# kalenforn/clip-based-cross-modal-hash

Measured on AMD Instinct MI355X. Metric: Hamming query x gallery pairs/sec (fused mAP@all pass, DCMHT COCO-shaped 64-bit), higher is better.
Workload: dtype u32; 1 GPU; configs[1] DCMHT COCO 64-bit retrieval: Q=5000 queries x R=117218 gallery items per GPU (x1 GPUs, contiguous shards), K=64 bits, C=80 classes, mAP@all; Q=5000, R_per_gpu=117218, K=64, C=80, parallelism=gallery-shard x1, query_blocks=1

## Files before the change

### clip-based-cross-modal-hash_amd/csrc/xmh_scan.hip

```cpp
#include "xmh_common.h"
#include <atomic>
#include <math.h>
#include <mutex>
#include <string.h>
#include <vector>
#include "xmh_scan_bits.h"
#include "xmh_scan_mfma.h"
#include "xmh_scan_kernels.h"

#include <stdlib.h>
#include <type_traits>

namespace {

constexpr int kSlotBudget64 = 9 * 1024;
constexpr int kSlotBudget32 = 5 * 1024;
constexpr int slots_for(int W, bool tern, int counter_bytes) {
    const int nbmax = (tern ? 64 : 32) * W + 1;
    const int budget = counter_bytes == 8 ? kSlotBudget64 : kSlotBudget32;
    const int cap = W > 8 ? 64 : 8;
    int S = 2;
    while (S < cap && nbmax * (64 / S) * counter_bytes > budget) S *= 2;
    return S;
}
// ... 62 lines not shown
WsLayout ws_layout(const xmh_scan_plan& p, size_t cache_bytes) {
    WsLayout L;
    const size_t cells = (size_t)p.nchunk * p.nbuckets * p.qpad;
    size_t o = 0;
    auto take = [&](size_t bytes) {
        const size_t at = o;
        o += (bytes + 255) & ~(size_t)255;
        return at;
    };
    L.chunk_hist = take(cells * 4);
    L.below = take(cells * 8);
    L.tot = take((size_t)p.nbuckets * p.qpad * 8);
    L.dpre = take((size_t)p.nbuckets * p.qpad * 8);
    L.cap = take((size_t)p.qpad * 4);
    L.tick = take((size_t)p.nqtile * 4);
    L.gate = take(256 + 8 * 4096);
    L.ap_part = take((size_t)p.nchunk * p.qpad * 4);
    L.pair_cache = take(cache_bytes);
    L.total = o;
    return L;
}

size_t cache_for_workspace(const xmh_scan_plan& p, int K, bool ternary, Family f, size_t ws_bytes) {
    const size_t c = pair_cache_bytes(p, K, ternary, f);
    return c && ws_bytes < ws_layout(p, c).total ? 0 : c;
}

int make_plan(int64_t Q, int64_t R, int K, int ternary, xmh_scan_plan* p, const Overrides& ov = {}) {
    if (Q <= 0 || R <= 0 || K <= 0) return xmh::fail(XMH_EINVAL, "scan plan: bad shape Q=%lld R=%lld K=%d", (long long)Q, (long long)R, K);
    if (R >= (1ll << 24) || Q >= (1ll << 24)) return xmh::fail(XMH_ENOTSUP, "scan plan: shard too large (R=%lld, Q=%lld)", (long long)R, (long long)Q);
    const int64_t nb = ternary ? 2 * (int64_t)K + 1 : (int64_t)K + 1;
    const int Wd = (K + 31) / 32;
    if (Wd > 64 || (ternary && Wd > 8))
        return xmh::fail(XMH_ENOTSUP, "scan plan: K=%d%s (at most 2048 code bits, 256 with zero planes)", K, ternary ? " ternary" : "");
    const int S64 = slots_for(instance_words(Wd), ternary != 0, 8);
    const int64_t lds_ap = nb * (64 / S64) * 8;
    if (lds_ap > 150 * 1024) return xmh::fail(XMH_ENOTSUP, "scan plan: %lld distance buckets need %lld B of LDS per wave; K=%d%s", (long long)nb, (long long)lds_ap, K, ternary ? " ternary" : "");
    const Family fam = pass1_family(K, ternary != 0, ov);
    const bool r2 = fam == Family::kR2 || fam == Family::kR2w;
    int64_t nqt = xmh::ceil_div(Q, 64);
    const int r2q = r2_geom(K).queries();
    if (r2) {
        int64_t l = r2q;
        while (l % 64) l += r2q;
        nqt = xmh::ceil_div(nqt * 64, l) * l / 64;
    }
    const int64_t wpc = 8;
    const int64_t slots = (int64_t)xmh::device_cu_count() * wpc;
    const bool cache_shape = !ternary && K > 32 && K <= 64 && cache_cap_mb() > 0;
    const int64_t rounds = nb <= 33 ? 3 : (nb <= 65 && !cache_shape ? 2 : 1);
    int64_t nchunk = rounds * slots / nqt;
    if (S64 > 8) nchunk = nchunk * 8 / S64;
    const bool mfma = fam != Family::kValu;
    if (mfma) {
        int64_t bsets = nb <= 129 ? 6 : 3;
        if (const char* e = xmh_experiment_env("XMH_BITS_SETS")) bsets = atoi(e) > 0 ? atoi(e) : bsets;
        nchunk = bsets * xmh::device_cu_count() / nqt;
        if (r2) {
            int sets = K > 32 && K <= 64 ? 1 : 2;
            if (const char* e = xmh_experiment_env("XMH_R2_SETS")) sets = atoi(e) > 0 ? atoi(e) : sets;
            nchunk = (int64_t)sets * xmh::device_cu_count() * r2_geom(K).blocks_per_cu / (nqt * 64 / r2q);
        }
    }
    if (nchunk < 1) nchunk = 1;
    if (nchunk > 8) nchunk = (nchunk + 4) / 8 * 8;
    int64_t chunk = xmh::ceil_div(R, nchunk);
    if (chunk < kMinChunk) chunk = kMinChunk;
    if (chunk > kMaxChunk) chunk = kMaxChunk;
    chunk = xmh::ceil_div(chunk, 8) * 8;
    if (mfma) {
        chunk = xmh::ceil_div(chunk, 64) * 64;
        int64_t bits_max = kBitsMaxChunk;
        if (const char* e = xmh_experiment_env("XMH_BITS_MAX_CHUNK")) bits_max = atoll(e) / 64 * 64 > 0 ? atoll(e) / 64 * 64 : bits_max;
        if (!r2 && chunk > bits_max) {
            nchunk = xmh::ceil_div(xmh::ceil_div(R, bits_max), 8) * 8;
            chunk = xmh::ceil_div(xmh::ceil_div(R, nchunk), 64) * 64;
        }
    }
    nchunk = xmh::ceil_div(R, chunk);
    p->chunk = chunk;
    p->nchunk = nchunk;
    p->nqtile = nqt;
    p->qpad = nqt * 64;
    p->nbuckets = nb;
    p->ws_bytes = ws_layout(*p, pair_cache_bytes(*p, K, ternary != 0, fam)).total;
    return XMH_OK;
}

int lane_order_ok(hipStream_t st) {
    static int cached[64];
    static bool have[64];
    static std::mutex mu;
    int dev = 0;
    if (hipGetDevice(&dev) != hipSuccess || dev < 0 || dev >= 64) return 0;
    if (getenv("XMH_SCAN_MASKED") != nullptr) return 0;
    std::lock_guard<std::mutex> lock(mu);
    if (have[dev]) return cached[dev];
    int ok = 0;
    {
        const char* fe = getenv("XMH_SCAN_PROBE_FAULT");
        const int fault = fe && atoi(fe) != 0;
        uint32_t* flag = nullptr;
        float* sink = nullptr;
        if (hipMalloc(&flag, 8) == hipSuccess && hipMalloc(&sink, 256) == hipSuccess) {
            uint32_t h[2] = {0, 1};
            int cus = xmh::device_cu_count();
            if (hipMemsetAsync(flag, 0, 8, st) == hipSuccess) {
                hipLaunchKernelGGL(k_probe_lane_order, dim3(1), dim3(64), 0, st, flag);
                hipLaunchKernelGGL(k_probe_lane_order_load, dim3((unsigned)(cus * 25)), dim3(64), 0, st, flag + 1, fault, sink);
                if (hipGetLastError() == hipSuccess && hipMemcpyAsync(h, flag, 8, hipMemcpyDeviceToHost, st) == hipSuccess && hipStreamSynchronize(st) == hipSuccess)
                    ok = h[0] == 1u && h[1] == 0u;
            }
        }
        if (flag) (void)hipFree(flag);
        if (sink) (void)hipFree(sink);
        if (!ok)
            fprintf(stderr, "xmh: the lane-order probe FAILED on device %d%s: same-address returning LDS adds are not served in lane order here; "
                            "pass 2 runs the masked kernels (about 2x slower, same results).\n", dev, fault ? " (XMH_SCAN_PROBE_FAULT set: forced)" : "");
// ... 134 lines not shown
    s.kern = Kern::kApS; s.W = tb ? 8 : W; s.LW = LW; s.tern = tern && !tb; s.masked = masked;
    s.cache = cache && !byte128 && !masked && pair_cache_shape(s.W, s.tern);
    s.stand_in = byte128 && apc;
    s.gate = size_gate | (s.stand_in ? kByWrap : 0u) | (r.rank_bits ? kByWidth : 0u);
    for (const bool p32 : {true, false}) {
        if (p32 ? r.rank_bits == 0 : apc16) continue;
        s.p32 = p32;
        s.S = s.cache ? cache_slots(s.W) : slots_for(s.W, s.tern, p32 ? 4 : 8);
        s.NW = s.S == 64 ? waves_for(s.W, s.tern) : 1;
        r.p2[r.n2++] = s;
    }
    return r;
}

int describe_launch(const Launch& l, char* out, size_t n) {
    static const char* const tf[2] = {"false", "true"};
    auto exists = [&](auto tern_c) { return dispatch_shape<decltype(tern_c)::value>(l.W, l.LW, [](auto, auto) { return (int)XMH_OK; }); };
    switch (l.kern) {
    case Kern::kHistS:
    case Kern::kApS:
        if (const int rc = l.tern ? exists(std::true_type{}) : exists(std::false_type{})) return rc;
        if (l.kern == Kern::kHistS) snprintf(out, n, "k_scan_hist_s<%d, %d, %s, %d, %d, %s>", l.W, l.LW, tf[l.tern], l.S, l.NW, tf[l.cache]);
        else
            snprintf(out, n, "k_scan_ap_s<%d, %d, %s, %s, %d, %s, %s, %d, %s>", l.W, l.cache ? 1 : l.LW, tf[l.tern], tf[!l.cache], l.S, tf[l.p32], tf[l.masked],
                     l.NW, tf[l.cache]);
        break;
    case Kern::kHistR2:
    case Kern::kHistR2w:
        snprintf(out, n, "k_scan_hist_%s<%d, %d, %d, %s>", l.kern == Kern::kHistR2 ? "r2" : "r2w", l.nml, l.NW, l.S, tf[l.cache]);
        break;
    case Kern::kHistB: {
        int nsh, nqt;
        xmh::scan_hist_bits_shape(l.S, l.tern, &nsh, &nqt);
        snprintf(out, n, "k_scan_hist_b<%d, %d, %d, %d, %s, %s>", l.S, kMfmaWaves, nsh, nqt, tf[l.cache], tf[l.tern]);
        break;
    }
    case Kern::kApC: snprintf(out, n, "k_scan_ap_c<false, %d, %s>", l.eb, tf[l.half]); break;
    case Kern::kApR2: snprintf(out, n, "k_scan_ap_r2<%d, %d, %d, false>", l.nml, l.NW, l.S); break;
    }
    return XMH_OK;
}

int check_common(const char* who, const ScanCall& c, const xmh_scan_plan& p) {
    if (!c.qbits || !c.rbits || !c.qlab || !c.rlab || !c.ws) return xmh::fail(XMH_EINVAL, "%s: null pointer", who);
    if ((c.qzero == nullptr) != (c.rzero == nullptr)) return xmh::fail(XMH_EINVAL, "%s: zero masks must be given for both sides or neither", who);
    if (c.C <= 0) return xmh::fail(XMH_EINVAL, "%s: C=%d", who, c.C);
    const size_t need = ws_layout(p, 0).total;
    if (c.ws_bytes < need) return xmh::fail(XMH_EINVAL, "%s: workspace too small (%zu < %zu; %zu with the pair cache)", who, c.ws_bytes, need, (size_t)p.ws_bytes);
    return XMH_OK;
}

ScanArgs make_args(const ScanCall& c, const xmh_scan_plan& p) {
    return ScanArgs{c.qbits, c.qzero, c.qlab, c.rbits, c.rzero, c.rlab, (int)c.Q, (int)c.R, c.K, (int)p.chunk, (int)p.nchunk, (int)p.nqtile, (int)p.qpad,
                    (int)p.nbuckets, nullptr};
}

MfmaArgs r2_args(const ScanCall& c, const Launch& l, const xmh_scan_plan& p, int nqt) {
    MfmaArgs a{c.qbits, (int)c.Q, (int)c.R, c.K, l.W, (int)p.chunk, (int)p.nchunk, nqt, (int)p.nbuckets, (int)p.qpad};
    a.rbits = c.rbits; a.rlab = c.rlab; a.qlab = c.qlab; a.LW = l.LW;
    return a;
}

struct Geom { unsigned grid, block; size_t lds; int nqt; };
Geom launch_geom(const Launch& l, const xmh_scan_plan& p) {
    const size_t nb = (size_t)p.nbuckets;
    const bool ap = l.kern == Kern::kApS || l.kern == Kern::kApC || l.kern == Kern::kApR2;
    Geom g{0, 64u * (unsigned)l.NW, 0, 0};
    if (l.kern == Kern::kHistS || l.kern == Kern::kApS) {
        g.lds = ((nb * (64 / l.S) * (ap && !l.p32 ? 2 : 1) + 3) & ~(size_t)3) * 4 * l.NW + (ap && l.cache ? 0 : aos_ring_bytes(l.W, l.LW, l.tern));
        g.nqt = (int)p.nqtile * l.S / l.NW;
    } else if (l.kern == Kern::kApC) {
        g.lds = nb * (64 / l.S) * 8; g.nqt = (int)p.nqtile * l.S;
    } else if (l.kern == Kern::kHistB) {
        g.nqt = (int)(p.qpad / (16 * kMfmaWaves));
    } else {
        g.lds = (size_t)l.NW * l.S * nb * 16 * (ap ? 8 : 4); g.nqt = (int)(p.qpad / (l.NW * l.S * 16));
    }
    g.grid = (unsigned)(8 * g.nqt * xmh::ceil_div(p.nchunk, 8));
    return g;
}

template <typename KernT, typename... Args>
int start(const char* who, const Launch& l, const Geom& g, hipStream_t st, KernT kern, int S, int NW, bool cache, Args... args) {
    if (l.S != S || l.NW != NW || l.cache != cache)
        return xmh::fail(XMH_ENOTSUP, "%s: the route names an instance with S=%d NW=%d cache=%d, the one compiled for W=%d LW=%d has S=%d NW=%d cache=%d", who, l.S,
                         l.NW, (int)l.cache, l.W, l.LW, S, NW, (int)cache);
    if (const int rc = xmh::raise_dynamic_lds(reinterpret_cast<const void*>(kern), g.lds, who)) return rc;
    hipLaunchKernelGGL(kern, dim3(g.grid), dim3(g.block), g.lds, st, args...);
    return XMH_OK;
}

struct ScanCtx {
    const ScanCall& c;
    hipStream_t st;
    xmh_scan_plan p;
    ScanRoute r;
    WsLayout L;
    ScanArgs a;
    uint32_t kcap = 0xffffffffu;
    bool capped = false;
    template <typename T> T* at(size_t off) const { return reinterpret_cast<T*>(static_cast<char*>(c.ws) + off); }
    uint32_t* chunk_hist() const { return at<uint32_t>(L.chunk_hist); }
    const uint2* below() const { return at<uint2>(L.below); }
    uint2* tot() const { return at<uint2>(L.tot); }
    uint2* dpre() const { return at<uint2>(L.dpre); }
    uint32_t* cap_ws() const { return at<uint32_t>(L.cap); }
    float* ap_part() const { return at<float>(L.ap_part); }
    ScanArgs args(const Geom& g, bool cached) const { ScanArgs as = a; as.nqt = g.nqt; as.pair_cache = cached ? pair_cache() : nullptr; return as; }
    uint32_t* gate(int word = 0) const { return at<uint32_t>(L.gate) + word; }
    const uint32_t* gate_if(const Launch& l, unsigned g, int word) const { return (l.gate & g) ? gate(word) : nullptr; }
    uint4* pair_cache() const { return r.cache_bytes ? at<uint4>(L.pair_cache) : nullptr; }
};

int plan_call(const char* who, ScanCtx& x, const Overrides& ov) {
    if (const int rc = make_plan(x.c.Q, x.c.R, x.c.K, x.c.tern, &x.p, ov)) return rc;
    return check_common(who, x.c, x.p);
}
void route_call(ScanCtx& x, Mode mode, const Overrides& ov) {
    x.r = scan_route(x.p, x.c, mode, ov, x.st);
    x.a = make_args(x.c, x.p);
    x.L = ws_layout(x.p, x.r.cache_bytes);
}

int valu_hist(const ScanCtx& x) {
    const Launch& h = x.r.p1;
    const Geom g = launch_geom(h, x.p);
    const ScanArgs as = x.args(g, h.cache);
    auto go = [&](auto kern, int S, int NW, bool cache) {
        xmh::ProfScope prof("scan_hist", x.st);
        return start("xmh_hamming_hist", h, g, x.st, kern, S, NW, cache, as, x.chunk_hist());
    };
    auto launch = [&](auto tern_c) {
        constexpr bool T = decltype(tern_c)::value;
        return dispatch_shape<T>(h.W, h.LW, [&](auto w, auto l) {
            constexpr int WW = decltype(w)::value, LL = decltype(l)::value;
            if constexpr (kPairCacheShape<WW, T>) {
                if (h.cache) return go(k_scan_hist_s<WW, LL, T, cache_slots(WW), 1, true>, cache_slots(WW), 1, true);
            }
            constexpr int S = slots_for(WW, T, 4);
            constexpr int NW = S == 64 ? waves_for(WW, T) : 1;
            return go(k_scan_hist_s<WW, LL, T, S, NW, false>, S, NW, false);
        });
    };
    return h.tern ? launch(std::true_type{}) : launch(std::false_type{});
}

int mfma_hist(const ScanCtx& x) {
    const Launch& h = x.r.p1;
    const xmh_scan_plan& p = x.p;
    const Geom g = launch_geom(h, p);
    uint32_t* chunk_hist = x.chunk_hist();
    uint4* cache = x.pair_cache();
    if (h.kern == Kern::kHistB) {
        xmh::ScanBitsArgs a{x.c.rbits, x.c.rlab, x.c.qbits, x.c.qlab, (int)x.c.Q, (int)x.c.R, x.c.K, h.W, h.LW, (int)p.chunk, (int)p.nchunk, g.nqt,
                            (int)p.nbuckets, (int)p.qpad};
        a.rzero = x.c.rzero; a.qzero = x.c.qzero;
        return xmh::launch_scan_hist_bits(a, h.S, chunk_hist, cache, x.st);
    }
    hipLaunchKernelGGL(k_scan_touch, dim3((unsigned)(8 * kTouchPerChunk * xmh::ceil_div(p.nchunk, 8))), dim3(256), 0, x.st, x.c.rbits, x.c.rlab, x.c.R, h.W, h.LW,
                       p.chunk, (int)p.nchunk, x.at<uint32_t>(x.L.tick), (int)((x.L.gate + 256 - x.L.tick) / 4));
    XMH_LAUNCH_CHECK("xmh_hamming_hist control words");
    const MfmaArgs a = r2_args(x.c, h, p, g.nqt);
    xmh::ProfScope prof("scan_hist", x.st);
    auto go = [&](auto kern, int NW, int NQ, bool cached, auto... wrap_word) { return start("xmh_hamming_hist", h, g, x.st, kern, NQ, NW, cached, a, chunk_hist, cache, wrap_word...); };
    if (h.kern == Kern::kHistR2w) {
        uint32_t* ovf = x.gate(kGateWrapped);
        return h.nml == 1 ? (h.cache ? go(k_scan_hist_r2w<1, 4, 2, true>, 4, 2, true, ovf) : go(k_scan_hist_r2w<1, 4, 2, false>, 4, 2, false, ovf))
                          : (h.cache ? go(k_scan_hist_r2w<2, 4, 2, true>, 4, 2, true, ovf) : go(k_scan_hist_r2w<2, 4, 2, false>, 4, 2, false, ovf));
    }
    return h.nml == 1 ? (h.cache ? go(k_scan_hist_r2<1, 4, 4, true>, 4, 4, true) : go(k_scan_hist_r2<1, 4, 4, false>, 4, 4, false))
                      : (h.cache ? go(k_scan_hist_r2<2, 4, 4, true>, 4, 4, true) : go(k_scan_hist_r2<2, 4, 4, false>, 4, 4, false));
}

int hamming_hist_impl(const ScanCall& c, uint32_t* hist_all, uint32_t* hist_rel, xmh_stream_t stream, const Overrides& ov) {
    ScanCtx x{c, xmh::as_stream(stream)};
    if (const int rc = plan_call("xmh_hamming_hist", x, ov)) return rc;
    route_call(x, Mode::kUnsharded, ov);
    const xmh_scan_plan& p = x.p;
    const Kern kern = x.r.p1.kern;
    if (kern == Kern::kHistS || kern == Kern::kHistB) XMH_HIP(hipMemsetAsync(x.at<char>(x.L.tick), 0, x.L.gate + 256 - x.L.tick, x.st));
    if (const int rc = kern == Kern::kHistS ? valu_hist(x) : mfma_hist(x)) return rc;
    XMH_LAUNCH_CHECK("xmh_hamming_hist");
    hipLaunchKernelGGL(k_scan_below, dim3((unsigned)p.nqtile, (unsigned)xmh::ceil_div(p.nbuckets, 4)), dim3(256), 0, x.st, x.chunk_hist(), (int)p.qpad,
                       (int)p.nbuckets, (int)p.nchunk, kern != Kern::kHistS ? kRelHi16 : 0u, x.at<uint2>(x.L.below), x.tot(), x.at<uint32_t>(x.L.tick), (int)c.Q, x.dpre(),
                       x.cap_ws(), x.gate(), hist_all, hist_rel);
    XMH_LAUNCH_CHECK("xmh_hamming_hist below");
    return XMH_OK;
}

}

extern "C" int xmh_scan_plan_make(int64_t Q, int64_t R, int K, int ternary, xmh_scan_plan* plan_host) {
    if (!plan_host) return xmh::fail(XMH_EINVAL, "xmh_scan_plan_make: null plan");
    return make_plan(Q, R, K, ternary, plan_host);
}

extern "C" size_t xmh_scan_pair_cache_bytes(int64_t Q, int64_t R, int K, int ternary) {
    xmh_scan_plan p;
    if (make_plan(Q, R, K, ternary, &p)) return 0;
    return pair_cache_bytes(p, K, ternary != 0, pass1_family(K, ternary != 0, {}));
}

extern "C" size_t xmh_scan_pair_cache_offset(int64_t Q, int64_t R, int K, int ternary) {
    xmh_scan_plan p;
    if (make_plan(Q, R, K, ternary, &p)) return (size_t)-1;
    return ws_layout(p, 0).pair_cache;
}

extern "C" size_t xmh_scan_ws_bytes_nocache(int64_t Q, int64_t R, int K, int ternary) {
    xmh_scan_plan p;
    if (make_plan(Q, R, K, ternary, &p)) return 0;
    return ws_layout(p, 0).total;
}

extern "C" int xmh_scan_describe(int64_t Q, int64_t R, int K, int C, int ternary, char* out, size_t out_bytes) {
    if (!out || out_bytes < 64) return xmh::fail(XMH_EINVAL, "xmh_scan_describe: buffer too small");
    xmh_scan_plan p;
    if (const int rc = make_plan(Q, R, K, ternary, &p)) return rc;
    Overrides ov;
    ov.describe = true;
    const ScanCall c{nullptr, nullptr, nullptr, nullptr, nullptr, nullptr, Q, R, K, C, nullptr, (size_t)p.ws_bytes, ternary != 0};
    const ScanRoute r = scan_route(p, c, Mode::kUnsharded, ov, nullptr);
    char p1[160], p2[200] = "", one[120];
    if (const int rc = describe_launch(r.p1, p1, sizeof(p1))) return rc;
    for (const bool p32 : {true, false})
        for (int i = 0; i < r.n2; ++i) {
            if (r.p2[i].stand_in || r.p2[i].p32 != p32) continue;
            if (const int rc = describe_launch(r.p2[i], one, sizeof(one))) return rc;
            const size_t at = strlen(p2);
            snprintf(p2 + at, sizeof(p2) - at, "%s%s", at ? "|" : "", one);
        }
    if ((size_t)snprintf(out, out_bytes, "pass1=%s;pass2=%s", p1, p2) >= out_bytes) return xmh::fail(XMH_EINVAL, "xmh_scan_describe: buffer too small");
    return XMH_OK;
}

extern "C" int xmh_hamming_hist(const uint32_t* qbits, const uint32_t* qzero, const uint32_t* qlab,
                                const uint32_t* rbits, const uint32_t* rzero, const uint32_t* rlab, int64_t Q, int64_t R,
                                int K, int C, void* ws, size_t ws_bytes, uint32_t* hist_all, uint32_t* hist_rel,
                                xmh_stream_t stream) {
    XMH_RANGE("xmh_hamming_hist (pass 1)");
    const ScanCall c{qbits, qzero, qlab, rbits, rzero, rlab, Q, R, K, C, ws, ws_bytes, qzero != nullptr};
    return hamming_hist_impl(c, hist_all, hist_rel, stream, {});
}

namespace {
int ap_offsets(const ScanCtx& x, const Pass2& o) {
    const xmh_scan_plan& p = x.p;
    if (o.mode == Mode::kUnsharded) return XMH_OK;
    if (o.mode == Mode::kAllToAll)
        hipLaunchKernelGGL(k_shard_scatter_offsets, dim3((unsigned)xmh::ceil_div(p.qpad, 256), (unsigned)p.nbuckets + 1), dim3(256), 0, x.st,
                           reinterpret_cast<const uint2*>(o.hist_g), (int)p.nbuckets, (int)(p.qpad / o.world), (int)x.c.Q, (int)p.qpad, o.k, x.dpre(), x.cap_ws(),
                           o.cap, x.gate(2));
    else if (o.mode == Mode::kTotals)
        hipLaunchKernelGGL(k_shard_offsets_dpre, dim3((unsigned)p.nqtile), dim3(256), 0, x.st, reinterpret_cast<const uint2*>(o.hist_g), o.world, o.rank,
                           (int)x.c.Q, (int)p.qpad, (int)p.nbuckets, o.k, x.dpre(), x.cap_ws(), o.cap, x.gate(2));
    else
        hipLaunchKernelGGL(k_scan_dpre, dim3((unsigned)p.nqtile), dim3(256), 0, x.st, (const uint2*)x.tot(), (int)x.c.Q, (int)p.qpad, (int)p.nbuckets, o.base_all,
                           o.base_rel, o.nrel_total, o.k, x.dpre(), x.cap_ws(), o.cap, (uint32_t*)nullptr, (uint32_t*)nullptr, (uint32_t*)nullptr, x.gate(2));
    XMH_LAUNCH_CHECK(o.mode == Mode::kAllToAll ? "xmh_hamming_map_sharded_offsets scatter" : (o.mode == Mode::kTotals ? "xmh_hamming_map_sharded offsets" : "xmh_hamming_ap dpre"));
    return XMH_OK;
}

int ap_launch_c(const ScanCtx& x, const Launch& l) {
    const Geom g = launch_geom(l, x.p);
    const ScanArgs as = x.args(g, true);
    xmh::ProfScope prof("scan_ap", x.st);
    auto go = [&](auto kc, int S) {
        return start("xmh_hamming_ap", l, g, x.st, kc, S, 1, l.cache, as, x.below(), (const uint2*)x.dpre(), (const uint32_t*)x.cap_ws(), x.ap_part(),
                     x.gate_if(l, kBySize, 2), x.kcap, x.gate_if(l, kByWrap, kGateWrapped), x.gate_if(l, kByWidth, 0), l.gate & kByWidth ? x.r.rank_bits : 0);
    };
    if (l.eb == 16) return x.capped ? go(k_scan_ap_c<true, 16>, 8) : go(k_scan_ap_c<false, 16>, 8);
    if (l.half) return x.capped ? go(k_scan_ap_c<true, 8, true>, 8) : go(k_scan_ap_c<false, 8, true>, 8);
    return x.capped ? go(k_scan_ap_c<true, 8>, 4) : go(k_scan_ap_c<false, 8>, 4);
}

int ap_launch_r2(const ScanCtx& x, const Launch& l) {
    const Geom g = launch_geom(l, x.p);
    const MfmaArgs ma = r2_args(x.c, l, x.p, g.nqt);
    xmh::ProfScope prof("scan_ap", x.st);
    auto go = [&](auto kern) {
        return start("xmh_hamming_ap", l, g, x.st, kern, kAp2Groups, kAp2Waves, l.cache, ma, x.below(), (const uint2*)x.dpre(), (const uint32_t*)x.cap_ws(), x.ap_part(),
                     x.gate_if(l, kBySize, 2), x.kcap);
    };
    return l.nml == 1 ? (x.capped ? go(k_scan_ap_r2<1, kAp2Waves, kAp2Groups, true>) : go(k_scan_ap_r2<1, kAp2Waves, kAp2Groups, false>))
                      : (x.capped ? go(k_scan_ap_r2<2, kAp2Waves, kAp2Groups, true>) : go(k_scan_ap_r2<2, kAp2Waves, kAp2Groups, false>));
}

int ap_launch_s(const ScanCtx& x, const Launch& l) {
    const Geom g = launch_geom(l, x.p);
    const ScanArgs as = x.args(g, l.cache);
    auto go = [&](auto kern, int S, int NW, bool cache, const uint32_t* run_if) {
        xmh::ProfScope prof(l.p32 ? "scan_ap32" : "scan_ap", x.st);
        return start("xmh_hamming_ap", l, g, x.st, kern, S, NW, cache, as, x.below(), (const uint2*)x.dpre(), (const uint32_t*)x.cap_ws(), x.ap_part(),
                     (const uint32_t*)x.gate(), x.r.rank_bits, x.kcap, x.gate_if(l, kBySize, 2), run_if);
    };
    auto by_shape = [&](auto tern_c, auto cap_c, auto p32_c, auto masked_c) {
        constexpr bool T = decltype(tern_c)::value, CP = decltype(cap_c)::value, P32 = decltype(p32_c)::value, MK = decltype(masked_c)::value;
        return dispatch_shape<T>(l.W, l.LW, [&](auto w, auto lw) {
            constexpr int WW = decltype(w)::value, LL = decltype(lw)::value;
            if constexpr (P32 && MK) return xmh::fail(XMH_ENOTSUP, "xmh_hamming_ap: the masked fallback runs 64-bit counters only");
            else {
                if constexpr (kPairCacheShape<WW, T> && !MK) {
                    if (l.cache)
                        return go(k_scan_ap_s<WW, 1, T, CP, cache_slots(WW), P32, MK, 1, true>, cache_slots(WW), 1, true, nullptr);
                }
                (void)CP;
                constexpr int S = slots_for(WW, T, P32 ? 4 : 8);
                constexpr int NW = S == 64 ? waves_for(WW, T) : 1;
                return go(k_scan_ap_s<WW, LL, T, true, S, P32, MK, NW, false>, S, NW, false, x.gate_if(l, kByWrap, kGateWrapped));
            }
        });
    };
    using T1 = std::true_type; using T0 = std::false_type;
    auto by_mask = [&](auto t, auto c, auto w) { return l.masked ? by_shape(t, c, w, T1{}) : by_shape(t, c, w, T0{}); };
    auto by_width = [&](auto t, auto c) { return l.p32 ? by_mask(t, c, T1{}) : by_mask(t, c, T0{}); };
    auto by_cap = [&](auto t) { return x.capped ? by_width(t, T1{}) : by_width(t, T0{}); };
    return l.tern ? by_cap(T1{}) : by_cap(T0{});
}

int ap_reduce(const ScanCtx& x, const Pass2& o) {
    const int64_t Q = x.c.Q;
    const unsigned nred = (unsigned)xmh::ceil_div(Q, 64);
    if (o.map_out && nred <= 4096) {
        hipLaunchKernelGGL(k_ap_reduce_map, dim3(nred), dim3(256), 0, x.st, (const float*)x.ap_part(), (int)Q, (int)x.p.qpad, (int)x.p.nchunk,
                           (const uint32_t*)x.cap_ws(), x.kcap, o.cap, o.ap_sum, x.at<double>(x.L.gate + 256), x.gate(1), o.map_out);
        XMH_LAUNCH_CHECK("xmh_hamming_map reduce+finalize");
        return XMH_OK;
    }
    hipLaunchKernelGGL(k_ap_reduce, dim3(nred), dim3(256), 0, x.st, (const float*)x.ap_part(), (int)Q, (int)x.p.qpad, (int)x.p.nchunk, o.ap_sum,
                       o.mode != Mode::kUnsharded ? (const uint32_t*)nullptr : (const uint32_t*)x.cap_ws(), x.kcap, o.cap);
    XMH_LAUNCH_CHECK("xmh_hamming_ap reduce");
    if (o.map_out) {
        hipLaunchKernelGGL(k_map_finalize, dim3(1), dim3(256), 0, x.st, (const double*)o.ap_sum, (const int32_t*)o.cap, Q, o.map_out);
        XMH_LAUNCH_CHECK("xmh_hamming_map finalize");
    }
    return XMH_OK;
}

static std::atomic<int> g_verify{0};
constexpr int XMH_EVERIFY_CODE = -74;

int hamming_ap_impl(const ScanCall& c, const Pass2& o, xmh_stream_t stream, const Overrides& ov);
// ... 237 lines not shown
```

### clip-based-cross-modal-hash_amd/csrc/xmh_scan_mfma.h

```cpp
#pragma once
#include "xmh_common.h"
#include <type_traits>

namespace {

constexpr int kMaxChunk = 32768;
constexpr uint32_t kF23 = 0x4B000000u;
constexpr int64_t kFloatBitsMaxItems = (1ll << 23) - 3;
constexpr int kMinChunk = 256;

struct ScanArgs {
    const uint32_t* qbits;
    const uint32_t* qzero;
    const uint32_t* qlab;
    const uint32_t* rbits;
    const uint32_t* rzero;
    const uint32_t* rlab;
    int Q, R, K;
    int chunk, nchunk, nqt, qpad, nb;
    uint4* pair_cache;
};

__device__ __forceinline__ bool map_block(const ScanArgs& a, int& chunk_id, int& qtile) {
    const int b = blockIdx.x;
    const int xcd = b & 7;
    const int t = b >> 3;
    qtile = t % a.nqt;
    chunk_id = xcd + 8 * (t / a.nqt);
    return chunk_id < a.nchunk;
}

typedef int v4i __attribute__((ext_vector_type(4)));

struct MfmaArgs {
    const uint32_t* qbits;
    int Q, R, K, W;
    int chunk, nchunk, nqt, nb, qpad;
    const uint32_t* rbits = nullptr;
    const uint32_t* rlab = nullptr;
    const uint32_t* qlab = nullptr;
    int LW = 0;
};

__device__ __forceinline__ bool mfma_map_block(const MfmaArgs& a, int& chunk_id, int& qtile) {
    const int b = blockIdx.x;
    const int xcd = b & 7, t = b >> 3;
    qtile = t % a.nqt;
    chunk_id = xcd + 8 * (t / a.nqt);
    return chunk_id < a.nchunk;
}

__device__ __forceinline__ v4i label_query_f4(uint32_t w, uint32_t one) {
    v4i r;
#pragma unroll
    for (int j = 0; j < 4; ++j) r[j] = (int)(((w >> j) & 0x11111111u) * one);
    return r;
}
__device__ __forceinline__ v4i label_item_f4(uint32_t w) {
    return v4i{(int)(w & 0x11111111u), (int)(w & 0x22222222u), (int)(w & 0x44444444u), (int)((w >> 1) & 0x44444444u)};
}

template <int NML, int NW, int NQ, bool CACHE>
__device__ __forceinline__ void scan_hist_r2_body(const MfmaArgs& a, uint32_t* __restrict__ chunk_hist, uint4* __restrict__ pair_cache) {
    static_assert(NML == 1 || NML == 2, "one i8 label tile (at most 64 classes) or one FP4 label tile (65-128 classes)");
    constexpr bool F4 = NML == 2;
    constexpr int NMI = 2, NMQ = 3;
    constexpr bool REGS = true;
    extern __shared__ __attribute__((aligned(16))) uint32_t lds[];
    int chunk_id, qtile;
    if (!mfma_map_block(a, chunk_id, qtile)) return;
    const int lane = threadIdx.x & 63, wave = threadIdx.x >> 6;
    const int ql = lane & 15, slot = lane >> 4;
    const int t16 = (qtile * NW + wave) * NQ;
    const int ncell = a.nb * 16;
    uint32_t* cnt = lds + (wave * NQ) * ncell;
    for (int e = lane; e < NQ * ncell; e += 64) cnt[e] = 0u;
    v4i bq[NQ][NMQ], cq[NQ], kqv[REGS ? NQ : 1];
    bool valid[NQ];
    const int rsh = 4 * (slot & 1), rwi = slot >> 1;
#pragma unroll
    for (int h = 0; h < NQ; ++h) {
        valid[h] = (t16 + h) * 16 + ql < a.Q;
        int pcq = 0;
        {
            const int64_t q = (int64_t)(t16 + h) * 16 + ql;
            uint32_t qw = 0u;
            if (valid[h]) {
                for (int w = 0; w < a.W; ++w) pcq += __popc(a.qbits[q * a.W + w]);
                if (rwi < a.W) qw = a.qbits[q * a.W + rwi];
            }
            qw >>= rsh;
#pragma unroll
            for (int j = 0; j < 4; ++j) {
                const uint32_t t = (qw >> j) & 0x01010101u;
                const bool on = valid[h] && rwi < a.W;
                if (j & 1) {
                    bq[h][0][j] = on ? (int)(0x20202020u ^ (t * 0xc0u)) : 0;
                    bq[h][1][j] = on ? (int)(0x01010101u ^ (t * 0xfeu)) : 0;
                } else {
                    bq[h][0][j] = on ? (int)(0x40404040u ^ (t << 7)) : 0;
                    bq[h][1][j] = on ? (int)(0x02020202u ^ (t * 0xfcu)) : 0;
                }
            }
            if constexpr (F4) {
                bq[h][2] = label_query_f4(valid[h] && slot < a.LW ? a.qlab[q * a.LW + slot] : 0u, 0x2u);
            } else {
                uint32_t lw = 0u;
                if (valid[h] && rwi < a.LW) lw = a.qlab[q * a.LW + rwi];
                lw >>= rsh;
#pragma unroll
                for (int j = 0; j < 4; ++j) bq[h][2][j] = (int)((lw >> j) & 0x01010101u);
            }
            const int k2 = 2 * pcq;
            kqv[h] = v4i{k2, k2, k2, k2};
        }
        const int c0 = (int)(uint32_t)(uintptr_t)(__attribute__((address_space(3))) uint32_t*)(cnt + h * ncell) + ql * 4 + (valid[h] ? 64 * pcq : 0);
        cq[h] = v4i{c0, c0, c0, c0};
    }
    v4i lab0 = {0x10000, 0x10000, 0x10000, 0x10000};
    asm volatile("" : "+v"(lab0));
#pragma unroll
    for (int h = 0; h < NQ; ++h) asm volatile("" : "+v"(cq[h]));
#pragma unroll
// ... 206 lines not shown
        build(A[3], wcur[3]);
#ifdef XMH_ABL_NOBUILD
        }
#endif
        group(std::integral_constant<int, 0>{});
        group(std::integral_constant<int, 1>{});
        group(std::integral_constant<int, 2>{});
        group(std::integral_constant<int, 3>{});
        asm volatile(XMH_R2_TAIL ::: "memory");
        consume(cw[NQ - 1][3], A[3]);
#ifdef XMH_ABL_NOSTORE
        if (CACHE && a.Q < 0) {
#else
        if (CACHE) {
#endif
#pragma unroll
            for (int h = 0; h < NQ; ++h) {
                uint4* dst = crow[h] + (int64_t)i * 64;
                __builtin_nontemporal_store(cw[h][0], &dst->x);
                __builtin_nontemporal_store(cw[h][1], &dst->y);
                __builtin_nontemporal_store(cw[h][2], &dst->z);
                __builtin_nontemporal_store(cw[h][3], &dst->w);
            }
        }
#pragma unroll
        for (int g = 0; g < 4; ++g)
#pragma unroll
            for (int m = 0; m < NMI; ++m) wcur[g][m] = wnxt[g][m];
    }
    const int npad = nbat * 64 - (int)(hi - lo);
    asm volatile("s_waitcnt lgkmcnt(0)" ::: "memory");
    if (npad > 0 && slot == 0) {
#pragma unroll
        for (int h = 0; h < NQ; ++h) {
            if (!valid[h]) continue;
            const int64_t q = (int64_t)(t16 + h) * 16 + ql;
            int dpad = 0;
            for (int w = 0; w < a.W; ++w) dpad += __popc(a.qbits[q * a.W + w]);
            cnt[h * ncell + dpad * 16 + ql] -= (uint32_t)npad << 16;
        }
    }
#pragma unroll
    for (int h = 0; h < NQ; ++h) {
        uint32_t* __restrict__ out = chunk_hist + ((int64_t)chunk_id * a.nb) * a.qpad + (t16 + h) * 16;
        for (int e = lane; e < ncell; e += 64) out[(int64_t)(e >> 4) * a.qpad + (e & 15)] = cnt[h * ncell + e];
    }
}

constexpr int kTouchPerChunk = 8;
__global__ __launch_bounds__(256) void k_scan_touch(const uint32_t* __restrict__ rbits, const uint32_t* __restrict__ rlab, int64_t R, int W, int LW, int64_t chunk,
                                                    int nchunk, uint32_t* __restrict__ ctl, int ctl_words) {
    if (blockIdx.x == 0)
        for (int e = threadIdx.x; e < ctl_words; e += 256) ctl[e] = 0u;
    const int b = blockIdx.x;
    const int c = (b & 7) + 8 * ((b >> 3) / kTouchPerChunk), sub = (b >> 3) % kTouchPerChunk;
    if (c >= nchunk) return;
    const int64_t lo = (int64_t)c * chunk, hi = lo + chunk < R ? lo + chunk : R;
    uint32_t acc = 0u;
    auto sweep = [&](const uint32_t* base, int64_t w0, int64_t w1) {
        for (int64_t w = w0 + ((int64_t)sub * 256 + threadIdx.x) * 32; w < w1; w += (int64_t)kTouchPerChunk * 256 * 32) acc ^= base[w];
    };
    sweep(rbits, lo * W, hi * W);
    sweep(rlab, lo * LW, hi * LW);
    asm volatile("" ::"v"(acc));
}

#ifndef XMH_R2_ATTR
#define XMH_R2_ATTR
#endif
template <int NML, int NW, int NQ, bool CACHE>
__global__ __launch_bounds__(64 * NW) XMH_R2_ATTR void k_scan_hist_r2(MfmaArgs a, uint32_t* __restrict__ chunk_hist, uint4* __restrict__ pair_cache) {
    scan_hist_r2_body<NML, NW, NQ, CACHE>(a, chunk_hist, pair_cache);
}

#define XMH_W_MFMA(D, A, B, C) "v_mfma_i32_16x16x64_i8 %[" D "], %[" A "], %[" B "], %[" C "]\n\t"
#define XMH_W_MFMA_F4(D, A, B, C) "v_mfma_f32_16x16x128_f8f6f4 %[" D "], %[" A "], %[" B "], %[" C "] cbsz:4 blgp:4\n\t"
#define XMH_W_MIN(I, L) "v_min_u32 %[" I "], 0x10001, %[" L "]\n\t"
#define XMH_W_ADD(A, D) "ds_add_u32 %[" A "], %[" D "]\n\t"
#define XMH_W_FUSED_CACHE(LAB) \
    asm volatile("s_nop 3\n\t" LAB("lab", "al0", "bl0", "lab0") XMH_W_MIN("i0", "lp0") XMH_W_MIN("i1", "lp1") XMH_W_MIN("i2", "lp2")                \
                 XMH_W_MIN("i3", "lp3") XMH_W_ADD("ap0", "i0") XMH_W_MFMA("addr", "a0", "ba0", "cq") XMH_W_ADD("ap1", "i1")                         \
                 XMH_W_MFMA("addr", "a1", "ba1", "addr") XMH_W_ADD("ap2", "i2") XMH_W_MFMA("d2", "a0", "bd0", "kq") XMH_W_ADD("ap3", "i3")          \
                 XMH_W_MFMA("d2", "a1", "bd1", "d2")                                                                                                \
                 : [lab] "=&v"(lab), [addr] "=&v"(addr), [d2] "=&v"(d2), [i0] "=&v"(i0), [i1] "=&v"(i1), [i2] "=&v"(i2), [i3] "=&v"(i3)             \
                 : [a0] "v"(At[0]), [a1] "v"(At[1]), [al0] "v"(At[2]), [ba0] "v"(bA[h][0]), [ba1] "v"(bA[h][1]), [bd0] "v"(bD[h][0]),               \
                   [bd1] "v"(bD[h][1]), [bl0] "v"(bL[h]), [lab0] "v"(lab0), [cq] "v"(cq[h]), [kq] "v"(kq[h]), [lp0] "v"(lab_p[0]),                  \
                   [lp1] "v"(lab_p[1]), [lp2] "v"(lab_p[2]), [lp3] "v"(lab_p[3]), [ap0] "v"(addr_p[0]), [ap1] "v"(addr_p[1]), [ap2] "v"(addr_p[2]), \
                   [ap3] "v"(addr_p[3])                                                                                                             \
                 : "memory")
#define XMH_W_FUSED_PLAIN(LAB) \
    asm volatile("s_nop 3\n\t" LAB("lab", "al0", "bl0", "lab0") XMH_W_MIN("i0", "lp0") XMH_W_MIN("i1", "lp1") XMH_W_MIN("i2", "lp2")                 \
                 XMH_W_MIN("i3", "lp3") XMH_W_ADD("ap0", "i0") XMH_W_ADD("ap1", "i1") XMH_W_MFMA("addr", "a0", "ba0", "cq") XMH_W_ADD("ap2", "i2")   \
                 XMH_W_ADD("ap3", "i3") XMH_W_MFMA("addr", "a1", "ba1", "addr")                                                                      \
                 : [lab] "=&v"(lab), [addr] "=&v"(addr), [i0] "=&v"(i0), [i1] "=&v"(i1), [i2] "=&v"(i2), [i3] "=&v"(i3)                              \
                 : [a0] "v"(At[0]), [a1] "v"(At[1]), [al0] "v"(At[2]), [ba0] "v"(bA[h][0]), [ba1] "v"(bA[h][1]), [bl0] "v"(bL[h]), [lab0] "v"(lab0), \
                   [cq] "v"(cq[h]), [lp0] "v"(lab_p[0]), [lp1] "v"(lab_p[1]), [lp2] "v"(lab_p[2]), [lp3] "v"(lab_p[3]), [ap0] "v"(addr_p[0]),        \
                   [ap1] "v"(addr_p[1]), [ap2] "v"(addr_p[2]), [ap3] "v"(addr_p[3])                                                                  \
                 : "memory")
template <int NML, int NW, int NQ, bool CACHE>
__global__ __launch_bounds__(64 * NW) void k_scan_hist_r2w(MfmaArgs a, uint32_t* __restrict__ chunk_hist, uint4* __restrict__ pair_cache,
                                                           uint32_t* __restrict__ ovf) {
    static_assert(NML == 1 || NML == 2, "one i8 label tile (at most 64 classes) or one FP4 label tile (65-128 classes)");
    constexpr bool F4 = NML == 2;
    constexpr int NMC = 2, NMI = NMC + 1;
    extern __shared__ __attribute__((aligned(16))) uint32_t lds[];
    int chunk_id, qtile;
    if (!mfma_map_block(a, chunk_id, qtile)) return;
    const int lane = threadIdx.x & 63, wave = threadIdx.x >> 6;
    const int ql = lane & 15, slot = lane >> 4;
    const int t16 = (qtile * NW + wave) * NQ;
    const int ncell = a.nb * 16;
    uint32_t* cnt = lds + (wave * NQ) * ncell;
    for (int e = lane; e < NQ * ncell; e += 64) cnt[e] = 0u;
    const int rsh = 4 * (slot & 1), rwi = slot >> 1;
    v4i bA[NQ][NMC], bD[NQ][NMC], bL[NQ], cq[NQ], kq[NQ];
    bool valid[NQ];
#pragma unroll
    for (int h = 0; h < NQ; ++h) {
        const int64_t q = (int64_t)(t16 + h) * 16 + ql;
        valid[h] = q < a.Q;
        int pcq = 0;
        if (valid[h])
            for (int w = 0; w < a.W; ++w) pcq += __popc(a.qbits[q * a.W + w]);
#pragma unroll
        for (int c = 0; c < NMC; ++c) {
            const int wi = 2 * c + rwi;
            const bool on = valid[h] && wi < a.W;
            const uint32_t qw = (on ? a.qbits[q * a.W + wi] : 0u) >> rsh;
#pragma unroll
            for (int j = 0; j < 4; ++j) {
                const uint32_t t = (qw >> j) & 0x01010101u;
                if (j & 1) {
                    bA[h][c][j] = on ? (int)(0x20202020u ^ (t * 0xc0u)) : 0;
                    bD[h][c][j] = on ? (int)(0x01010101u ^ (t * 0xfeu)) : 0;
                } else {
                    bA[h][c][j] = on ? (int)(0x40404040u ^ (t << 7)) : 0;
                    bD[h][c][j] = on ? (int)(0x02020202u ^ (t * 0xfcu)) : 0;
                }
            }
        }
        if constexpr (F4) {
            bL[h] = label_query_f4(valid[h] && slot < a.LW ? a.qlab[q * a.LW + slot] : 0u, 0x2u);
        } else {
            uint32_t lw = 0u;
            if (valid[h] && rwi < a.LW) lw = a.qlab[q * a.LW + rwi];
            lw >>= rsh;
#pragma unroll
            for (int j = 0; j < 4; ++j) bL[h][j] = (int)((lw >> j) & 0x01010101u);
        }
        const int c0 = (int)(uint32_t)(uintptr_t)(__attribute__((address_space(3))) uint32_t*)(cnt + h * ncell) + ql * 4 + (valid[h] ? 64 * pcq : 0);
        const int k2 = valid[h] ? 2 * pcq : 0;
        cq[h] = v4i{c0, c0, c0, c0};
        kq[h] = v4i{k2, k2, k2, k2};
    }
    v4i lab0 = {0x10000, 0x10000, 0x10000, 0x10000};
    asm volatile("" : "+v"(lab0));
#pragma unroll
    for (int h = 0; h < NQ; ++h) asm volatile("" : "+v"(cq[h]), "+v"(kq[h]));
    const int64_t lo = (int64_t)chunk_id * a.chunk;
    const int64_t hi = (lo + a.chunk < a.R) ? lo + a.chunk : a.R;
// ... 395 lines not shown
            issue4(oldB, mB, r3);
            r3 = words_at(bi + 7);
            drain8(oldA, mA);
            drain0(oldB, mB);
        }
        const int rem = nfull - bi;
        if (rem >= 2) {
            issue4(oldA, mA, r0);
            issue4(oldB, mB, r1);
            drain8(oldA, mA);
            drain0(oldB, mB);
            if (rem == 3) {
                issue4(oldA, mA, r2);
                drain0(oldA, mA);
            }
        } else if (rem == 1) {
            issue4(oldA, mA, r0);
            drain0(oldA, mA);
        }
        cw = rem == 0 ? r0 : (rem == 1 ? r1 : (rem == 2 ? r2 : r3));
    }
    const int cntb = (int)(hi - lo) - nfull * 64;
    slow_batch(cw, cntb);
#pragma unroll
    for (int o = QW; o < 64; o <<= 1) acc += __shfl_xor(acc, o, 64);
    if (slot == 0) ap_part[(int64_t)chunk_id * a.qpad + q] = acc;
}

#define XMH_AP2_SETA "v113", "v115", "v117", "v119", "v[112:113]", "v[114:115]", "v[116:117]", "v[118:119]"
#define XMH_AP2_SETB "v121", "v123", "v125", "v127", "v[120:121]", "v[122:123]", "v[124:125]", "v[126:127]"
#define XMH_AP2_MFMA(D, A, B, C) "v_mfma_i32_16x16x64_i8 %[" D "], %[" A "], %[" B "], " C "\n\t"
#define XMH_AP2_MFMA_F4(D, A, B, C) "v_mfma_f32_16x16x128_f8f6f4 %[" D "], %[" A "], %[" B "], " C " cbsz:4 blgp:4\n\t"
#define XMH_AP2_MAX(H, L) "v_max_i32 " H ", -1, %[" L "]\n\t"
#define XMH_AP2_ADD(O, A, P) "ds_add_rtn_u64 %[" O "], %[" A "], " P "\n\t"
#define XMH_AP2_FUSED_(LAB, H0, H1, H2, H3, P0, P1, P2, P3)                                                                              \
    "s_nop 3\n\t" LAB("lab", "a1", "q1", "0") XMH_AP2_MAX(H0, "l0") XMH_AP2_MAX(H1, "l1") XMH_AP2_MAX(H2, "l2") XMH_AP2_MAX(H3, "l3")    \
    XMH_AP2_MFMA("addr", "a0", "q0", "%[c0]") XMH_AP2_ADD("o0", "p0", P0) XMH_AP2_ADD("o1", "p1", P1) XMH_AP2_ADD("o2", "p2", P2)       \
    XMH_AP2_ADD("o3", "p3", P3)
#define XMH_AP2_TAIL_(H0, H1, H2, H3, P0, P1, P2, P3)                                                                                     \
    XMH_AP2_MAX(H0, "l0") XMH_AP2_MAX(H1, "l1") XMH_AP2_MAX(H2, "l2") XMH_AP2_MAX(H3, "l3") XMH_AP2_ADD("o0", "p0", P0)                   \
    XMH_AP2_ADD("o1", "p1", P1) XMH_AP2_ADD("o2", "p2", P2) XMH_AP2_ADD("o3", "p3", P3)
#define XMH_AP2_FUSED(...) XMH_AP2_FUSED_(__VA_ARGS__)
#define XMH_AP2_TAIL(...) XMH_AP2_TAIL_(__VA_ARGS__)
template <int NML, int NW, int NQ, bool CAPPED>
__global__ __launch_bounds__(64 * NW) void k_scan_ap_r2(MfmaArgs a, const uint2* __restrict__ below, const uint2* __restrict__ dpre,
                                                        const uint32_t* __restrict__ cap_ws, float* __restrict__ ap_part,
                                                        const uint32_t* __restrict__ items_total, uint32_t kcap) {
    using u64 = unsigned long long;
    static_assert(NML == 1 || NML == 2, "one i8 label tile (at most 64 classes) or one FP4 label tile (65-128 classes)");
    constexpr bool F4 = NML == 2;
    constexpr int NMI = 2;
    extern __shared__ __attribute__((aligned(16))) uint32_t lds[];
    int chunk_id, qtile;
    if (!mfma_map_block(a, chunk_id, qtile)) return;
    if (items_total && (int64_t)*items_total > kFloatBitsMaxItems) return;
    const int lane = threadIdx.x & 63, wave = threadIdx.x >> 6;
    const int ql = lane & 15, slot = lane >> 4;
    const int t16 = (qtile * NW + wave) * NQ;
    const int ncell = a.nb * 16;
    u64* cnt = reinterpret_cast<u64*>(lds) + (wave * NQ) * ncell;
    auto pack = [](uint2 x, uint2 y) {
        return (u64)(kF23 + x.x + y.x + 1u) | ((u64)(kF23 + (0x7fffffu - (x.y + y.y + 1u))) << 32);
    };
#pragma unroll
    for (int h = 0; h < NQ; ++h) {
        const uint2* __restrict__ pb = below + ((int64_t)chunk_id * a.nb) * a.qpad + (t16 + h) * 16;
        const uint2* __restrict__ pd = dpre + (t16 + h) * 16;
        u64* c = cnt + h * ncell;
        auto cell = [&](int e) { return e; };
        int e = lane;
        for (; e + 3 * 64 < ncell; e += 4 * 64) {
            uint2 x[4], y[4];
#pragma unroll
            for (int j = 0; j < 4; ++j) {
                const int ee = e + j * 64;
                const int64_t at = (int64_t)(ee >> 4) * a.qpad + (ee & 15);
                x[j] = pb[at];
                y[j] = pd[at];
            }
#pragma unroll
            for (int j = 0; j < 4; ++j) c[cell(e + j * 64)] = pack(x[j], y[j]);
        }
        for (; e < ncell; e += 64) {
            const int64_t at = (int64_t)(e >> 4) * a.qpad + (e & 15);
            c[cell(e)] = pack(pb[at], pd[at]);
        }
    }
    v4i bq[NQ], bl[NQ], cq[NQ];
    float capf[NQ], acc[NQ];
    const int rsh = 4 * (slot & 1), rwi = slot >> 1;
#pragma unroll
    for (int h = 0; h < NQ; ++h) {
        const int64_t q = (int64_t)(t16 + h) * 16 + ql;
        const bool valid = q < a.Q;
        int pcq = 0;
        uint32_t qw = 0u;
        if (valid) {
            for (int w = 0; w < a.W; ++w) pcq += __popc(a.qbits[q * a.W + w]);
            if (rwi < a.W) qw = a.qbits[q * a.W + rwi];
        }
        qw >>= rsh;
        const bool on = valid && rwi < a.W;
#pragma unroll
        for (int j = 0; j < 4; ++j) {
            const uint32_t t = (qw >> j) & 0x01010101u;
            if (j & 1) bq[h][j] = on ? (int)(0x20202020u ^ (t * 0xc0u)) : 0;
            else bq[h][j] = on ? (int)(0x40404040u ^ (t << 7)) : 0;
// ... 184 lines not shown
```

Before: 1761 billion pairs/s.

## Map blocks exactly to chunks and skip all-padding query tiles in AP pass

Replaces the XCD-strided block mapping, which rounded the grid up to a multiple of 8 chunks and launched idle blocks, with a shared map that covers whole groups of 8 chunks XCD-strided and then places the remaining tail chunks linearly. The AP launches now size their grid to the query tiles that actually contain queries rather than all padded tiles, so blocks on padding do no work. An opt-in env flag also lets the R2 plan keep a non-multiple-of-8 chunk count. The tail chunks lose the XCD-aligned placement, which may hurt L2 locality for them, and the touch kernel uses a single part per tail chunk.

```diff
diff --git a/clip-based-cross-modal-hash_amd/csrc/xmh_scan.hip b/clip-based-cross-modal-hash_amd/csrc/xmh_scan.hip
--- a/clip-based-cross-modal-hash_amd/csrc/xmh_scan.hip
+++ b/clip-based-cross-modal-hash_amd/csrc/xmh_scan.hip
@@ -138,6 +138,7 @@
     int64_t nchunk = rounds * slots / nqt;
     if (S64 > 8) nchunk = nchunk * 8 / S64;
     const bool mfma = fam != Family::kValu;
+    bool fill = false;
     if (mfma) {
         int64_t bsets = nb <= 129 ? 6 : 3;
         if (const char* e = xmh_experiment_env("XMH_BITS_SETS")) bsets = atoi(e) > 0 ? atoi(e) : bsets;
@@ -146,10 +147,11 @@
             int sets = K > 32 && K <= 64 ? 1 : 2;
             if (const char* e = xmh_experiment_env("XMH_R2_SETS")) sets = atoi(e) > 0 ? atoi(e) : sets;
             nchunk = (int64_t)sets * xmh::device_cu_count() * r2_geom(K).blocks_per_cu / (nqt * 64 / r2q);
+            if (const char* e = xmh_experiment_env("XMH_R2_FILL")) fill = atoi(e) != 0 && fam == Family::kR2 && sets == 1 && cache_shape && ap_r2_mode() != 1;
         }
     }
     if (nchunk < 1) nchunk = 1;
-    if (nchunk > 8) nchunk = (nchunk + 4) / 8 * 8;
+    if (nchunk > 8 && !fill) nchunk = (nchunk + 4) / 8 * 8;
     int64_t chunk = xmh::ceil_div(R, nchunk);
     if (chunk < kMinChunk) chunk = kMinChunk;
     if (chunk > kMaxChunk) chunk = kMaxChunk;
@@ -390,7 +392,7 @@
 
 ScanArgs make_args(const ScanCall& c, const xmh_scan_plan& p) {
     return ScanArgs{c.qbits, c.qzero, c.qlab, c.rbits, c.rzero, c.rlab, (int)c.Q, (int)c.R, c.K, (int)p.chunk, (int)p.nchunk, (int)p.nqtile, (int)p.qpad,
-                    (int)p.nbuckets, nullptr};
+                    (int)p.nbuckets, nullptr, (int)p.nqtile};
 }
 
 MfmaArgs r2_args(const ScanCall& c, const Launch& l, const xmh_scan_plan& p, int nqt) {
@@ -399,8 +401,8 @@
     return a;
 }
 
-struct Geom { unsigned grid, block; size_t lds; int nqt; };
-Geom launch_geom(const Launch& l, const xmh_scan_plan& p) {
+struct Geom { unsigned grid, block; size_t lds; int nqt, nrun; };
+Geom launch_geom(const Launch& l, const xmh_scan_plan& p, int64_t Q) {
     const size_t nb = (size_t)p.nbuckets;
     const bool ap = l.kern == Kern::kApS || l.kern == Kern::kApC || l.kern == Kern::kApR2;
     Geom g{0, 64u * (unsigned)l.NW, 0, 0};
@@ -414,7 +416,12 @@
     } else {
         g.lds = (size_t)l.NW * l.S * nb * 16 * (ap ? 8 : 4); g.nqt = (int)(p.qpad / (l.NW * l.S * 16));
     }
-    g.grid = (unsigned)(8 * g.nqt * xmh::ceil_div(p.nchunk, 8));
+    g.nrun = g.nqt;
+    if (ap) {
+        static const bool all_tiles = xmh_experiment_env("XMH_AP_TILES") && atoi(xmh_experiment_env("XMH_AP_TILES")) == 0;
+        if (!all_tiles) g.nrun = (int)xmh::ceil_div(Q, p.qpad / g.nqt);
+    }
+    g.grid = xmh::scan_grid_blocks(g.nrun, (int)p.nchunk);
     return g;
 }
 
@@ -444,7 +451,7 @@
     uint2* dpre() const { return at<uint2>(L.dpre); }
     uint32_t* cap_ws() const { return at<uint32_t>(L.cap); }
     float* ap_part() const { return at<float>(L.ap_part); }
-    ScanArgs args(const Geom& g, bool cached) const { ScanArgs as = a; as.nqt = g.nqt; as.pair_cache = cached ? pair_cache() : nullptr; return as; }
+    ScanArgs args(const Geom& g, bool cached) const { ScanArgs as = a; as.nqt = g.nqt; as.nrun = g.nrun; as.pair_cache = cached ? pair_cache() : nullptr; return as; }
     uint32_t* gate(int word = 0) const { return at<uint32_t>(L.gate) + word; }
     const uint32_t* gate_if(const Launch& l, unsigned g, int word) const { return (l.gate & g) ? gate(word) : nullptr; }
     uint4* pair_cache() const { return r.cache_bytes ? at<uint4>(L.pair_cache) : nullptr; }
@@ -462,7 +469,7 @@
 
 int valu_hist(const ScanCtx& x) {
     const Launch& h = x.r.p1;
-    const Geom g = launch_geom(h, x.p);
+    const Geom g = launch_geom(h, x.p, x.c.Q);
     const ScanArgs as = x.args(g, h.cache);
     auto go = [&](auto kern, int S, int NW, bool cache) {
         xmh::ProfScope prof("scan_hist", x.st);
@@ -486,7 +493,7 @@
 int mfma_hist(const ScanCtx& x) {
     const Launch& h = x.r.p1;
     const xmh_scan_plan& p = x.p;
-    const Geom g = launch_geom(h, p);
+    const Geom g = launch_geom(h, p, x.c.Q);
     uint32_t* chunk_hist = x.chunk_hist();
     uint4* cache = x.pair_cache();
     if (h.kern == Kern::kHistB) {
@@ -495,7 +502,7 @@
         a.rzero = x.c.rzero; a.qzero = x.c.qzero;
         return xmh::launch_scan_hist_bits(a, h.S, chunk_hist, cache, x.st);
     }
-    hipLaunchKernelGGL(k_scan_touch, dim3((unsigned)(8 * kTouchPerChunk * xmh::ceil_div(p.nchunk, 8))), dim3(256), 0, x.st, x.c.rbits, x.c.rlab, x.c.R, h.W, h.LW,
+    hipLaunchKernelGGL(k_scan_touch, dim3(xmh::scan_grid_blocks(kTouchPerChunk, (int)p.nchunk)), dim3(256), 0, x.st, x.c.rbits, x.c.rlab, x.c.R, h.W, h.LW,
                        p.chunk, (int)p.nchunk, x.at<uint32_t>(x.L.tick), (int)((x.L.gate + 256 - x.L.tick) / 4));
     XMH_LAUNCH_CHECK("xmh_hamming_hist control words");
     const MfmaArgs a = r2_args(x.c, h, p, g.nqt);
@@ -600,7 +607,7 @@
 }
 
 int ap_launch_c(const ScanCtx& x, const Launch& l) {
-    const Geom g = launch_geom(l, x.p);
+    const Geom g = launch_geom(l, x.p, x.c.Q);
     const ScanArgs as = x.args(g, true);
     xmh::ProfScope prof("scan_ap", x.st);
     auto go = [&](auto kc, int S) {
@@ -613,8 +620,8 @@
 }
 
 int ap_launch_r2(const ScanCtx& x, const Launch& l) {
-    const Geom g = launch_geom(l, x.p);
-    const MfmaArgs ma = r2_args(x.c, l, x.p, g.nqt);
+    const Geom g = launch_geom(l, x.p, x.c.Q);
+    const MfmaArgs ma = r2_args(x.c, l, x.p, g.nrun);
     xmh::ProfScope prof("scan_ap", x.st);
     auto go = [&](auto kern) {
         return start("xmh_hamming_ap", l, g, x.st, kern, kAp2Groups, kAp2Waves, l.cache, ma, x.below(), (const uint2*)x.dpre(), (const uint32_t*)x.cap_ws(), x.ap_part(),
@@ -625,7 +632,7 @@
 }
 
 int ap_launch_s(const ScanCtx& x, const Launch& l) {
-    const Geom g = launch_geom(l, x.p);
+    const Geom g = launch_geom(l, x.p, x.c.Q);
     const ScanArgs as = x.args(g, l.cache);
     auto go = [&](auto kern, int S, int NW, bool cache, const uint32_t* run_if) {
         xmh::ProfScope prof(l.p32 ? "scan_ap32" : "scan_ap", x.st);
diff --git a/clip-based-cross-modal-hash_amd/csrc/xmh_scan_map.h b/clip-based-cross-modal-hash_amd/csrc/xmh_scan_map.h
--- /dev/null
+++ b/clip-based-cross-modal-hash_amd/csrc/xmh_scan_map.h
@@ -0,0 +1,21 @@
+#pragma once
+
+namespace xmh {
+
+__host__ __device__ inline unsigned scan_grid_blocks(int ntile, int nchunk) { return (unsigned)ntile * (unsigned)nchunk; }
+
+__host__ __device__ inline bool scan_block_map(int b, int ntile, int nchunk, int& chunk_id, int& tile) {
+    const int whole = nchunk & ~7;
+    const int lb = b - whole * ntile;
+    if (lb < 0) {
+        const int t = b >> 3;
+        tile = t % ntile;
+        chunk_id = (b & 7) + 8 * (t / ntile);
+        return true;
+    }
+    tile = lb % ntile;
+    chunk_id = whole + lb / ntile;
+    return chunk_id < nchunk;
+}
+
+}
diff --git a/clip-based-cross-modal-hash_amd/csrc/xmh_scan_mfma.h b/clip-based-cross-modal-hash_amd/csrc/xmh_scan_mfma.h
--- a/clip-based-cross-modal-hash_amd/csrc/xmh_scan_mfma.h
+++ b/clip-based-cross-modal-hash_amd/csrc/xmh_scan_mfma.h
@@ -1,5 +1,6 @@
 #pragma once
 #include "xmh_common.h"
+#include "xmh_scan_map.h"
 #include <type_traits>
 
 namespace {
@@ -19,15 +20,11 @@
     int Q, R, K;
     int chunk, nchunk, nqt, qpad, nb;
     uint4* pair_cache;
+    int nrun;
 };
 
 __device__ __forceinline__ bool map_block(const ScanArgs& a, int& chunk_id, int& qtile) {
-    const int b = blockIdx.x;
-    const int xcd = b & 7;
-    const int t = b >> 3;
-    qtile = t % a.nqt;
-    chunk_id = xcd + 8 * (t / a.nqt);
-    return chunk_id < a.nchunk;
+    return xmh::scan_block_map((int)blockIdx.x, a.nrun, a.nchunk, chunk_id, qtile);
 }
 
 typedef int v4i __attribute__((ext_vector_type(4)));
@@ -42,12 +39,8 @@
     int LW = 0;
 };
 
-__device__ __forceinline__ bool mfma_map_block(const MfmaArgs& a, int& chunk_id, int& qtile) {
-    const int b = blockIdx.x;
-    const int xcd = b & 7, t = b >> 3;
-    qtile = t % a.nqt;
-    chunk_id = xcd + 8 * (t / a.nqt);
-    return chunk_id < a.nchunk;
+__device__ __forceinline__ bool map_block(const MfmaArgs& a, int& chunk_id, int& qtile) {
+    return xmh::scan_block_map((int)blockIdx.x, a.nqt, a.nchunk, chunk_id, qtile);
 }
 
 __device__ __forceinline__ v4i label_query_f4(uint32_t w, uint32_t one) {
@@ -68,7 +61,7 @@
     constexpr bool REGS = true;
     extern __shared__ __attribute__((aligned(16))) uint32_t lds[];
     int chunk_id, qtile;
-    if (!mfma_map_block(a, chunk_id, qtile)) return;
+    if (!map_block(a, chunk_id, qtile)) return;
     const int lane = threadIdx.x & 63, wave = threadIdx.x >> 6;
     const int ql = lane & 15, slot = lane >> 4;
     const int t16 = (qtile * NW + wave) * NQ;
@@ -381,13 +374,14 @@
                                                     int nchunk, uint32_t* __restrict__ ctl, int ctl_words) {
     if (blockIdx.x == 0)
         for (int e = threadIdx.x; e < ctl_words; e += 256) ctl[e] = 0u;
-    const int b = blockIdx.x;
-    const int c = (b & 7) + 8 * ((b >> 3) / kTouchPerChunk), sub = (b >> 3) % kTouchPerChunk;
-    if (c >= nchunk) return;
+    int c, sub;
+    if (!xmh::scan_block_map((int)blockIdx.x, kTouchPerChunk, nchunk, c, sub)) return;
+    const int parts = c < (nchunk & ~7) ? kTouchPerChunk : 1;
+    if (parts == 1) sub = 0;
     const int64_t lo = (int64_t)c * chunk, hi = lo + chunk < R ? lo + chunk : R;
     uint32_t acc = 0u;
     auto sweep = [&](const uint32_t* base, int64_t w0, int64_t w1) {
-        for (int64_t w = w0 + ((int64_t)sub * 256 + threadIdx.x) * 32; w < w1; w += (int64_t)kTouchPerChunk * 256 * 32) acc ^= base[w];
+        for (int64_t w = w0 + ((int64_t)sub * 256 + threadIdx.x) * 32; w < w1; w += (int64_t)parts * 256 * 32) acc ^= base[w];
     };
     sweep(rbits, lo * W, hi * W);
     sweep(rlab, lo * LW, hi * LW);
@@ -434,7 +428,7 @@
     constexpr int NMC = 2, NMI = NMC + 1;
     extern __shared__ __attribute__((aligned(16))) uint32_t lds[];
     int chunk_id, qtile;
-    if (!mfma_map_block(a, chunk_id, qtile)) return;
+    if (!map_block(a, chunk_id, qtile)) return;
     const int lane = threadIdx.x & 63, wave = threadIdx.x >> 6;
     const int ql = lane & 15, slot = lane >> 4;
     const int t16 = (qtile * NW + wave) * NQ;
@@ -936,7 +930,7 @@
     constexpr int NMI = 2;
     extern __shared__ __attribute__((aligned(16))) uint32_t lds[];
     int chunk_id, qtile;
-    if (!mfma_map_block(a, chunk_id, qtile)) return;
+    if (!map_block(a, chunk_id, qtile)) return;
     if (items_total && (int64_t)*items_total > kFloatBitsMaxItems) return;
     const int lane = threadIdx.x & 63, wave = threadIdx.x >> 6;
     const int ql = lane & 15, slot = lane >> 4;
```

New measurement: 1784 billion pairs/s, median of 6. 1.01x the previous value.
